# ducha-aiki/affnet

Hardware: NVIDIA H100
Metric: Mpix/s end-to-end HesAffNet(+OriNet)+HardNet (higher is better)
Workload: dtype fp16 operands (fp16 residual planes: AffNet/OriNet weights+activations, HardNet layer 2-3 weights), fp32 accumulate; stencils fp32

## Files before the change

affnet_b200/csrc/tcx_conv.cuh:

```cuda
#pragma once
#include <cuda_bf16.h>

#include "tc_conv.cuh"

#ifndef AG_CONV_PINGPONG
#define AG_CONV_PINGPONG 1
#endif

namespace ag {
namespace tcx {

using namespace ag::tc;

constexpr int XORDER = 5;

enum { CT_TOTAL, CT_WAIT_FULL, CT_TURN, CT_ISSUE, CT_MMA_WAIT, CT_EPILOGUE, CT_WG_BAR, CT_WAIT_EMPTY, CT_OTHER, CT_STATES };
#ifdef AG_CONV_TIMELINE
constexpr int CT_CTAS = 4, CT_LAUNCHES = 16, CT_EVENTS = 2048;
__device__ unsigned long long g_conv_tl[CT_LAUNCHES][CT_CTAS][9][CT_STATES];
__device__ unsigned long long g_conv_ev[CT_LAUNCHES][2][CT_EVENTS][3];
__device__ int g_conv_tl_launch[CT_CTAS];
struct ConvTimeline {
    unsigned long long t[CT_STATES];
    long long start, mark;
    int slot, warp, n_ev;
    __device__ static void claim(int* s_slot) {
        if (threadIdx.x == 0)
            *s_slot = (blockIdx.y == 0 && blockIdx.x < CT_CTAS) ? min(atomicAdd(&g_conv_tl_launch[blockIdx.x], 1), CT_LAUNCHES) : CT_LAUNCHES;
    }
    __device__ void init(const int* s_slot) {
        for (int i = 0; i < CT_STATES; i++) t[i] = 0;
        slot = *s_slot; warp = threadIdx.x >> 5; n_ev = 0;
        start = mark = clock64();
    }
    __device__ void lap(int state) { const long long now = clock64(); t[state] += (unsigned long long)(now - mark); mark = now; }
    __device__ void event(int k) {
        if (blockIdx.x == 0 && slot < CT_LAUNCHES && (threadIdx.x & 127) == 0 && n_ev < CT_EVENTS) g_conv_ev[slot][warp >> 2][n_ev][k] = (unsigned long long)mark;
        if (k == 2) n_ev++;
    }
    __device__ void finish() {
        t[CT_TOTAL] = (unsigned long long)(clock64() - start);
        if ((threadIdx.x & 31) == 0 && slot < CT_LAUNCHES)
            for (int i = 0; i < CT_STATES; i++) g_conv_tl[slot][blockIdx.x][warp][i] = t[i];
    }
};
#else
struct ConvTimeline {
    __device__ static void claim(int*) {}
    __device__ void init(const int*) {}
    __device__ void lap(int) {}
    __device__ void event(int) {}
    __device__ void finish() {}
};
#endif

enum XLayout { L_S2_16 = 0, L_S1_16 = 1, L_S2_8P = 2, L_S1_8P = 3, L_HEAD = 4 };

__device__ __forceinline__ void bulk_g2s_mc(void* dst, const void* src, uint32_t bytes, uint64_t* bar, uint16_t mask) {
    asm volatile("cp.async.bulk.shared::cluster.global.mbarrier::complete_tx::bytes.multicast::cluster [%0], [%1], %2, [%3], %4;" ::"r"(smem_u32(dst)),
                 "l"(src), "r"(bytes), "r"(smem_u32(bar)), "h"(mask)
                 : "memory");
}
__device__ __forceinline__ void mbar_arrive_cluster(uint64_t* bar, uint32_t cta) {
    asm volatile("{\n .reg .b32 ra;\n mapa.shared::cluster.u32 ra, %0, %1;\n mbarrier.arrive.release.cta.shared::cluster.b64 _, [ra];\n}\n" ::"r"(smem_u32(bar)), "r"(cta)
                 : "memory");
}
__device__ __forceinline__ void cluster_sync() {
    asm volatile("barrier.cluster.arrive.release.aligned;\n barrier.cluster.wait.acquire.aligned;" ::: "memory");
}

template <int BF>
__device__ __forceinline__ uint32_t pack2(float a, float b) {
    if (BF) { const __nv_bfloat162 h = __floats2bfloat162_rn(a, b); return *reinterpret_cast<const uint32_t*>(&h); }
    const __half2 h = __floats2half2_rn(a, b);
    return *reinterpret_cast<const uint32_t*>(&h);
}
template <int BF>
__device__ __forceinline__ float2 unpack2(uint32_t u) {
    if (BF) return make_float2(__uint_as_float(u << 16), __uint_as_float(u & 0xFFFF0000u));
    return __half22float2(*reinterpret_cast<const __half2*>(&u));
}
template <int LO, int BF = 0>
__device__ __forceinline__ void split_pack8(const float* v, uint4& hi, uint4& lo) {
    uint32_t h[4], l[4];
#pragma unroll
    for (int i = 0; i < 4; i++) {
        h[i] = pack2<BF>(v[2 * i], v[2 * i + 1]);
        if (LO) {
            const float2 f = unpack2<BF>(h[i]);
            l[i] = pack2<BF>(v[2 * i] - f.x, v[2 * i + 1] - f.y);
        } else l[i] = 0;
    }
    hi = make_uint4(h[0], h[1], h[2], h[3]);
    lo = make_uint4(l[0], l[1], l[2], l[3]);
}

template <int LO, int BF = 0>
__device__ __forceinline__ void split_pack2(float v0, float v1, uint32_t& hi, uint32_t& lo) {
    hi = pack2<BF>(v0, v1);
    if (LO) {
        const float2 f = unpack2<BF>(hi);
        lo = pack2<BF>(v0 - f.x, v1 - f.y);
    } else lo = 0;
}

__host__ __device__ constexpr int layout_slots(int lay) { return lay == L_S2_16 ? 1024 : lay == L_S1_16 ? 256 : lay == L_S2_8P ? 512 : 128; }
__host__ __device__ constexpr int layout_pair(int lay) { return (lay == L_S2_8P || lay == L_S1_8P) ? 1 : 0; }
__host__ __device__ constexpr int rpos(int x) { return (x & 1) * 8 + (x >> 1); }
__host__ __device__ constexpr int ppos(int x, int p) { return (x & 1) * 8 + p * 4 + (x >> 1); }
__host__ __device__ constexpr int layout_slot(int lay, int y, int x, int p) {
    return lay == L_S2_16 ? ((y & 1) * 2 + (x & 1)) * 256 + (y >> 1) * 16 + rpos(x >> 1)
         : lay == L_S1_16 ? y * 16 + rpos(x)
         : lay == L_S2_8P ? ((y & 1) * 2 + (x & 1)) * 128 + (y >> 1) * 16 + ppos(x >> 1, p)
                          : y * 16 + ppos(x, p);
}

template <int H, int STRIDE>
struct XIn {
    static constexpr int HOUT = H / STRIDE;
    static constexpr int PAIR = (HOUT == 8) ? 1 : 0;
    static constexpr int W = HOUT;
    static constexpr int RW = W * (1 + PAIR);
    static constexpr int TILES = HOUT * RW / 128;
    static constexpr int NPLANES = (STRIDE == 1) ? 1 : 4;
    static constexpr int DATA = HOUT * RW;
    static constexpr int PLANE = DATA + RW;
    static constexpr int SLOT_STAGE = NPLANES * PLANE;
    static constexpr int LAYOUT = (STRIDE == 2) ? (PAIR ? L_S2_8P : L_S2_16) : (PAIR ? L_S1_8P : L_S1_16);
    static_assert(HOUT == 8 || HOUT == 16 || HOUT == 32, "map sizes of the three nets");
    static_assert(!(STRIDE == 1 && H == 32), "the 32x32 stride-1 layer lives in tcx_first.cuh");
};

struct XArgs {
    const __half* in;
    void* out;
    const __half* wpk;
    const float* bias;
    float inv_scale;
    int n, group;
    const int* count;
};

template <int CIN, int COUT, int H, int STRIDE, int NSPLIT, int STAGES, int OUT, int SA, int SW, int OSA>
struct XCfg {
    using In = XIn<H, STRIDE>;
    static constexpr int CO = COUT, STRD = STRIDE, OUTL = OUT, SPLIT_A = SA, SPLIT_W = SW, SPLIT_O = OSA;
    static constexpr int KC = CIN / 8, NT = COUT / NSPLIT, HOUT = In::HOUT;
    static constexpr int G = KC * (1 + SA);
    static constexpr int GS = STAGES * In::SLOT_STAGE + (STRIDE == 1 ? In::RW : 0);
    static constexpr int ACCW = 3 * NT;
    static constexpr int BLOCKS = 2 * In::TILES;
    static constexpr uint32_t W_BYTES = 9u * CIN * NT * 2u * (1 + SW);
    static constexpr uint32_t IN_BYTES = (uint32_t)G * GS * 16u;
    static constexpr uint32_t HI_IN_BYTES = (uint32_t)KC * In::NPLANES * In::DATA * 16u;
    static constexpr uint32_t UNIT_IN_BYTES = HI_IN_BYTES * (1 + SA);
    static constexpr int THREADS = 288;
    static constexpr size_t SMEM = 1024 + (size_t)W_BYTES + IN_BYTES;
    static constexpr size_t HI_OUT_BYTES = (size_t)(COUT / 8) * layout_slots(OUT) * 16;
    static constexpr size_t UNIT_OUT_BYTES = (OUT == L_HEAD) ? 0 : HI_OUT_BYTES * (1 + OSA);
    static constexpr int NR1 = (1 + SW) * 3 * NT;
    static constexpr int NRO = (1 + SW) * 2 * NT, NRE = (1 + SW) * NT;
    static_assert(CIN % 16 == 0 && NT % 16 == 0 && ACCW <= 256, "wgmma shape");
    static_assert(In::W == 8 || In::W == 16, "a warp's 16 accumulator rows hold whole image rows");
    static_assert(SA <= 1 && SW <= 1 && OSA <= 1, "split-precision switches are 0 | 1");
    static_assert(2 * STAGES + 1 <= 60, "barrier area");
    static_assert(SMEM <= 232448, "shared memory budget");
    static_assert(GS < 16384, "leading-byte offset field");
    static_assert(OUT == L_HEAD || layout_pair(OUT) || !In::PAIR, "a pair layer writes pair layouts or the head operand");
};

__device__ __forceinline__ float frag_left_even(float v1, int lane) { return __shfl_sync(0xffffffffu, v1, (lane + 28) & 31); }
__device__ __forceinline__ float frag_right_odd(float v0, int lane) { return __shfl_sync(0xffffffffu, v0, (lane + 4) & 31); }

__device__ __forceinline__ bool xpatch_valid(const XArgs& a, int pi) { return pi < a.n && (a.count == nullptr || (pi % a.group) < a.count[pi / a.group]); }

template <class Cfg, int BF>
__device__ __forceinline__ void xconv_block_issue(float* d, uint32_t a_t, uint32_t w_base) {
    using In = typename Cfg::In;
    constexpr int KC = Cfg::KC, NT = Cfg::NT, GS = Cfg::GS, RW = In::RW, SA = Cfg::SPLIT_A, SW = Cfg::SPLIT_W;
    constexpr uint32_t LBO_A = ((uint32_t)GS) << 16;
    wgmma_fence();
    if (Cfg::STRD == 1) {
#pragma unroll
        for (int dy = 0; dy < 3; dy++) {
#pragma unroll
            for (int j = 0; j < KC / 2; j++) {
                const uint32_t ahi = ((a_t + (uint32_t)(dy * RW + 2 * j * GS)) & 0x3FFFu) | LBO_A;
                const uint32_t alo = ((a_t + (uint32_t)(dy * RW + (KC + 2 * j) * GS)) & 0x3FFFu) | LBO_A;
                const uint32_t blk = w_base + (uint32_t)((dy * (KC / 2) + j) * 2 * Cfg::NR1);
                const uint32_t bhi = (blk & 0x3FFFu) | ((uint32_t)Cfg::NR1 << 16), blo = ((blk + 3 * NT) & 0x3FFFu) | ((uint32_t)Cfg::NR1 << 16);
                Wgmma<3 * NT, BF>::mma(d, desc64(ahi), desc64(bhi), (dy | j) != 0);
                if (SW) Wgmma<3 * NT, BF>::mma(d, desc64(ahi), desc64(blo), 1);
                if (SA) Wgmma<3 * NT, BF>::mma(d, desc64(alo), desc64(bhi), 1);
            }
        }
    } else {
#pragma unroll
        for (int dy = 0; dy < 3; dy++) {
            constexpr int PL = In::PLANE;
            const int py = (dy == 1) ? 0 : 1, ro = (dy == 0) ? 0 : 1;
#pragma unroll
            for (int j = 0; j < KC / 2; j++) {
                const uint32_t blk = w_base + (uint32_t)((dy * (KC / 2) + j) * 2 * (Cfg::NRO + Cfg::NRE));
                const uint32_t bo_hi = (blk & 0x3FFFu) | ((uint32_t)Cfg::NRO << 16), bo_lo = ((blk + 2 * NT) & 0x3FFFu) | ((uint32_t)Cfg::NRO << 16);
                const uint32_t be = blk + 2 * Cfg::NRO;
                const uint32_t be_hi = (be & 0x3FFFu) | ((uint32_t)Cfg::NRE << 16), be_lo = ((be + NT) & 0x3FFFu) | ((uint32_t)Cfg::NRE << 16);
                const uint32_t ao = a_t + (uint32_t)((py * 2 + 1) * PL + ro * RW);
                const uint32_t ao_hi = ((ao + (uint32_t)(2 * j * GS)) & 0x3FFFu) | LBO_A, ao_lo = ((ao + (uint32_t)((KC + 2 * j) * GS)) & 0x3FFFu) | LBO_A;
                Wgmma<2 * NT, BF>::mma(d, desc64(ao_hi), desc64(bo_hi), (dy | j) != 0);
                if (SW) Wgmma<2 * NT, BF>::mma(d, desc64(ao_hi), desc64(bo_lo), 1);
                if (SA) Wgmma<2 * NT, BF>::mma(d, desc64(ao_lo), desc64(bo_hi), 1);
                const uint32_t ae = a_t + (uint32_t)((py * 2 + 0) * PL + ro * RW);
                const uint32_t ae_hi = ((ae + (uint32_t)(2 * j * GS)) & 0x3FFFu) | LBO_A, ae_lo = ((ae + (uint32_t)((KC + 2 * j) * GS)) & 0x3FFFu) | LBO_A;
                Wgmma<NT, BF>::mma(d + NT, desc64(ae_hi), desc64(be_hi), (dy | j) != 0);
                if (SW) Wgmma<NT, BF>::mma(d + NT, desc64(ae_hi), desc64(be_lo), 1);
                if (SA) Wgmma<NT, BF>::mma(d + NT, desc64(ae_lo), desc64(be_hi), 1);
            }
        }
    }
    wgmma_commit();
}
template <class Cfg, int BF>
__device__ __forceinline__ void xconv_block_epilogue(const float* d, const XArgs& a, const float* s_bias, int u, int b, int split, int wq, int lane) {
    using In = typename Cfg::In;
    constexpr int NT = Cfg::NT, HOUT = Cfg::HOUT, W = In::W, PAIR = In::PAIR, COUT = Cfg::CO, OUT = Cfg::OUTL, OSA = Cfg::SPLIT_O;
    unsigned char* obase[2];
    bool ok[2];
    size_t lo_off = 0;
    const int i = lane >> 2, xi = PAIR ? (i & 3) : i;
    const bool has_l0 = xi > 0, has_r1 = xi < W / 2 - 1;
    static_assert(W == 16 || PAIR, "neighbour-paired row groups: 16 pixels, or 8 of each patch of a pair");
#pragma unroll
    for (int h = 0; h < 2; h++) {
        const int y = b * 4 + wq, x = 2 * xi + h, pi = PAIR ? 2 * u + (i >> 2) : u;
        ok[h] = xpatch_valid(a, pi);
        if (OUT == L_HEAD) {
            obase[h] = reinterpret_cast<unsigned char*>(a.out) + (((size_t)(pi >> 7) * (HOUT * HOUT * COUT / 8) + (size_t)(y * HOUT + x) * (COUT / 8)) * 128 + (pi & 127)) * 16;
            lo_off = (size_t)((a.n + 127) >> 7) * (HOUT * HOUT * COUT / 8) * 128 * 16;
        } else {
            const int ou = layout_pair(OUT) ? (pi >> 1) : pi;
            obase[h] = reinterpret_cast<unsigned char*>(a.out) + (size_t)ou * Cfg::UNIT_OUT_BYTES + (size_t)layout_slot(OUT, y, x, pi & 1) * 16;
            lo_off = (size_t)(COUT / 8) * layout_slots(OUT) * 16;
        }
    }
#pragma unroll
    for (int j = 0; j < NT / 8; j++) {
        const int c = j * 8 + 2 * (lane & 3);
        float v[2][2];
#pragma unroll
        for (int e = 0; e < 2; e++) {
            const float c00 = d[4 * j + e], c01 = d[4 * j + 2 + e];
            const float c10 = d[4 * (j + NT / 8) + e], c11 = d[4 * (j + NT / 8) + 2 + e];
            const float c20 = d[4 * (j + 2 * NT / 8) + e], c21 = d[4 * (j + 2 * NT / 8) + 2 + e];
            const float l0 = frag_left_even(c01, lane);
            float acc0, acc1;
            if (Cfg::STRD == 1) {
                const float r1 = frag_right_odd(c20, lane);
                const float t0 = c21 + c10, t1 = has_r1 ? r1 + c11 : c11;
                acc0 = has_l0 ? l0 + t0 : t0;
                acc1 = c00 + t1;
            } else {
                const float t0 = c10 + c20, t1 = c11 + c21;
                acc0 = has_l0 ? l0 + t0 : t0;
                acc1 = c00 + t1;
            }
            v[0][e] = fmaxf(fmaf(acc0, a.inv_scale, s_bias[c + e]), 0.f);
            v[1][e] = fmaxf(fmaf(acc1, a.inv_scale, s_bias[c + e]), 0.f);
        }
        const int ch = split * NT + c;
        const size_t goff = ((OUT == L_HEAD) ? (size_t)(ch / 8) * 128 * 16 : (size_t)(ch / 8) * layout_slots(OUT) * 16) + (ch & 7) * 2;
#pragma unroll
        for (int h = 0; h < 2; h++) {
            if (!ok[h]) continue;
            uint32_t hi, lo;
            split_pack2<OSA, BF>(v[h][0], v[h][1], hi, lo);
            *reinterpret_cast<uint32_t*>(obase[h] + goff) = hi;
            if (OSA) *reinterpret_cast<uint32_t*>(obase[h] + lo_off + goff) = lo;
        }
    }
}

template <int CIN, int COUT, int H, int STRIDE, int NSPLIT, int STAGES, int OUT, int SA, int SW, int OSA, int BF = 0, int MC = 0, int PPS = 0>
__global__ void __launch_bounds__(288, 1) tcx_conv_kernel(const XArgs a) {
    static_assert(MC == 0 || NSPLIT == 2, "multicast pairs the two channel-split CTAs");
    using Cfg = XCfg<CIN, COUT, H, STRIDE, NSPLIT, STAGES, OUT, SA, SW, OSA>;
    using In = typename Cfg::In;
    constexpr int ACCW = Cfg::ACCW, BLOCKS = Cfg::BLOCKS, GS = Cfg::GS, RW = In::RW;
    constexpr int PAIR = In::PAIR;
    constexpr bool PP = AG_CONV_PINGPONG && PPS;
    extern __shared__ __align__(1024) unsigned char smem[];
    uint64_t* full = reinterpret_cast<uint64_t*>(smem);
    uint64_t* empty = full + STAGES;
    uint64_t* wbar = empty + STAGES;
    float* s_bias = reinterpret_cast<float*>(smem + 512);
    unsigned char* sW = smem + 1024;
    unsigned char* sIn = sW + Cfg::W_BYTES;

    const int warp = threadIdx.x >> 5, lane = threadIdx.x & 31;
    const int split = blockIdx.y;
    const int n_units = PAIR ? (a.n + 1) >> 1 : a.n;

    int* s_tl_slot = reinterpret_cast<int*>(smem + 496);

    if (threadIdx.x < Cfg::NT) s_bias[threadIdx.x] = a.bias[split * Cfg::NT + threadIdx.x];
    if (threadIdx.x == 0) {
        for (int s = 0; s < STAGES; s++) { mbar_init(&full[s], 1); mbar_init(&empty[s], (PP ? 8 : 2) * (1 + MC)); }
        mbar_init(wbar, 1);
        asm volatile("fence.mbarrier_init.release.cluster;" ::: "memory");
    }
    ConvTimeline::claim(s_tl_slot);
    for (int i = threadIdx.x; i < (int)(Cfg::IN_BYTES / 16); i += blockDim.x) reinterpret_cast<uint4*>(sIn)[i] = make_uint4(0, 0, 0, 0);
    asm volatile("fence.proxy.async.shared::cta;" ::: "memory");
    __syncthreads();
    if (MC) cluster_sync();
    ConvTimeline tl;
    tl.init(s_tl_slot);
    auto release = [&](uint64_t* e) {
        if (MC) { mbar_arrive_cluster(e, 0); mbar_arrive_cluster(e, 1); }
        else mbar_arrive(e);
    };

    auto uvalid = [&](int u) -> bool { return PAIR ? (xpatch_valid(a, 2 * u) || xpatch_valid(a, 2 * u + 1)) : xpatch_valid(a, u); };

    if (warp == 8) {
        if (lane == 0) {
            mbar_expect_tx(wbar, Cfg::W_BYTES);
            bulk_g2s(sW, reinterpret_cast<const unsigned char*>(a.wpk) + (size_t)split * Cfg::W_BYTES, Cfg::W_BYTES, wbar);
            int it = 0;
            for (int u = blockIdx.x; u < n_units; u += gridDim.x) {
                if (!uvalid(u)) continue;
                const int s = it % STAGES;
                tl.lap(CT_OTHER);
                mbar_wait(&empty[s], ((it / STAGES) & 1) ^ 1);
                tl.lap(CT_WAIT_EMPTY);
                mbar_expect_tx(&full[s], Cfg::UNIT_IN_BYTES);
                const unsigned char* gsrc = reinterpret_cast<const unsigned char*>(a.in) + (size_t)u * Cfg::UNIT_IN_BYTES;
#pragma unroll 1
                for (int g = 0; g < Cfg::G; g++)
#pragma unroll
                    for (int pl = 0; pl < In::NPLANES; pl++) {
                        unsigned char* dst = sIn + ((size_t)g * GS + (size_t)s * In::SLOT_STAGE + (size_t)pl * In::PLANE + RW) * 16;
                        const unsigned char* srcp = gsrc + ((size_t)g * In::NPLANES + pl) * In::DATA * 16;
                        if (MC) { if (((g * In::NPLANES + pl) & 1) == split) bulk_g2s_mc(dst, srcp, In::DATA * 16u, &full[s], (uint16_t)3); }
                        else bulk_g2s(dst, srcp, In::DATA * 16u, &full[s]);
                    }
                it++;
            }
            tl.lap(CT_OTHER);
            if (MC) {
                for (int k = 0; k < STAGES && k < it; k++) { const int j = it - 1 - k; mbar_wait(&empty[j % STAGES], (j / STAGES) & 1); }
            }
            tl.lap(CT_WAIT_EMPTY);
        }
    } else if (warp < 8) {
        const int wg = warp >> 2, wq = warp & 3;
        mbar_wait(wbar, 0);
        const uint32_t w_base = smem_u32(sW) >> 4;
        const uint32_t in_base = smem_u32(sIn) >> 4;
        int it = 0;
        for (int u = blockIdx.x; u < n_units; u += gridDim.x) {
            if (!uvalid(u)) continue;
            const int s = it % STAGES;
            tl.lap(CT_OTHER);
            mbar_wait(&full[s], (it / STAGES) & 1);
            tl.lap(CT_WAIT_FULL);
            const uint32_t st_base = in_base + (uint32_t)(s * In::SLOT_STAGE);
#pragma unroll 1
            for (int b = wg; b < BLOCKS; b += 2) {
                float d[ACCW / 2];
                if (PP && (wg == 1 || it > 0 || b > 0)) bar_sync(XORDER + wg, 256);
                tl.lap(CT_TURN);
                tl.event(0);
                xconv_block_issue<Cfg, BF>(d, st_base + (uint32_t)(b * 64), w_base);
                if (PP) asm volatile("bar.arrive %0, 256;" ::"r"(XORDER + (wg ^ 1)) : "memory");
                tl.lap(CT_ISSUE);
                wgmma_wait<0>();
                wgmma_reg_fence<ACCW / 2>(d);
                tl.lap(CT_MMA_WAIT);
                tl.event(1);
                if (PP && b + 2 >= BLOCKS && lane == 0) release(&empty[s]);
                xconv_block_epilogue<Cfg, BF>(d, a, s_bias, u, b, split, wq, lane);
                tl.lap(CT_EPILOGUE);
                tl.event(2);
            }
            if (!PP) {
                bar_sync(3 + wg, 128);
                tl.lap(CT_WG_BAR);
                if ((threadIdx.x & 127) == 0) release(&empty[s]);
            }
            it++;
        }
        if (PP && wg == 0 && it > 0) bar_sync(XORDER, 256);
        tl.lap(CT_OTHER);
    }
    tl.finish();
    __syncthreads();
    if (MC) cluster_sync();
}

}
}
```

affnet_b200/csrc/tcx_first.cuh:

```cuda
#pragma once
#include "tcx_conv.cuh"

#ifdef AG_FIRST_TIMELINE
#define AG_TL(state, ...) do { const long long t_ = clock64(); __VA_ARGS__; tl[state] += (unsigned long long)(clock64() - t_); } while (0)
#else
#define AG_TL(state, ...) do { __VA_ARGS__; } while (0)
#endif

namespace ag {
namespace tcx {

enum { TL_TOTAL, TL_WAIT_P, TL_ISSUE, TL_MMA_WAIT, TL_WG_BAR, TL_STAGE_BAR, TL_PBUILD, TL_STATES };
#ifdef AG_FIRST_TIMELINE
constexpr int TL_CTAS = 4, TL_LAUNCHES = 8;
__device__ unsigned long long g_first_tl[TL_LAUNCHES][TL_CTAS][16][TL_STATES];
__device__ int g_first_tl_launch[TL_CTAS];
#endif

__device__ __forceinline__ void stmatrix_x4(const void* row, uint32_t r0, uint32_t r1, uint32_t r2, uint32_t r3) {
    asm volatile("stmatrix.sync.aligned.m8n8.x4.shared.b16 [%0], {%1, %2, %3, %4};" ::"r"(smem_u32(row)), "r"(r0), "r"(r1), "r"(r2), "r"(r3)
                 : "memory");
}

template <int C1, int COUT, int SA, int SW, int OSA, int L3 = 0>
struct XFirstCfg {
    using X3 = XCfg<COUT, 2 * COUT, 32, 2, 1, 1, L_S1_16, 1, 1, 1>;
    static constexpr int KC = C1 / 8, NT = COUT;
    static constexpr int BLOCKS = 16;
    static constexpr int NPIXP = 18 * 32;
    static constexpr int SX = 1200;
    static constexpr int S1 = (C1 == 16) ? 1 : 0;
    static constexpr int ACC1 = 32;
    static constexpr int ACCW = 3 * NT;
    static constexpr int G = KC * (1 + SA);
    static constexpr int SLOT_STAGE = 1024 + 32;
    static constexpr int NSTAGE = L3 ? 1 : 2;
    static constexpr int GS = NSTAGE * SLOT_STAGE + 32;
    static constexpr int NR = (1 + SW) * 3 * NT;
    static constexpr uint32_t W_BYTES = 9u * C1 * NT * 2u * (1 + SW);
    static constexpr uint32_t IN_BYTES = (uint32_t)G * GS * 16u;
    static constexpr uint32_t W1_BYTES = 2u * 2u * C1 * 16;
    static constexpr uint32_t P_BYTES = 2u * 2u * NPIXP * 16;
    static constexpr uint32_t XCH_BYTES = 2u * 2u * 4u * 2u * NT * 4u;
    static constexpr uint32_t W3_BYTES = L3 ? X3::W_BYTES : 0u;
    static constexpr uint32_t IN3_BYTES = L3 ? X3::IN_BYTES : 0u;
    static constexpr size_t SMEM = 1024 + (size_t)W_BYTES + W3_BYTES + IN_BYTES + IN3_BYTES + P_BYTES + W1_BYTES + 2 * SX * 4 + 256 + XCH_BYTES;
    static constexpr size_t HI_OUT_BYTES = (size_t)(COUT / 8) * 1024 * 16;
    static constexpr size_t UNIT_OUT_BYTES = HI_OUT_BYTES * (1 + OSA);
    static constexpr int THREADS = 512;
    static constexpr int REG_PRODUCER = 96, REG_CONSUMER = 160;
    static_assert(256 * (REG_PRODUCER + REG_CONSUMER) <= 65536 && REG_PRODUCER % 8 == 0 && REG_CONSUMER % 8 == 0, "register split");
    static_assert(BLOCKS % 4 == 0 && (!L3 || X3::BLOCKS == 4), "two blocks in flight per warpgroup: an even count of blocks each");
    static_assert(C1 % 16 == 0 && NT % 16 == 0 && ACCW <= 256, "shape");
    static_assert(SA <= 1 && SW <= 1 && OSA <= 1, "split-precision switches are 0 | 1");
    static_assert(!L3 || (OSA == 1 && X3::NT <= 32), "layer 3 reads hi + lo planes; its bias fits smem[640, 768)");
    static_assert(C1 == 16 || C1 == 32, "layer-1 accumulator width");
    static_assert(SA || KC % 2 == 0, "layer-1 epilogue: one stmatrix.x4 per channel group (hi + lo) or per two (hi only)");
    static_assert(SMEM <= 232448, "shared memory budget");
};

template <int C1, int COUT, int SA, int SW, int OSA, int BF = 0, int L3 = 0>
__global__ void __launch_bounds__(512, 1) tcx_first_kernel(const XArgs a, const FirstSrc src, const XArgs a3) {
    using Cfg = XFirstCfg<C1, COUT, SA, SW, OSA, L3>;
    using X3 = typename Cfg::X3;
    constexpr int KC = Cfg::KC, NT = Cfg::NT, ACCW = Cfg::ACCW, NPIXP = Cfg::NPIXP, SX = Cfg::SX, GS = Cfg::GS;
    extern __shared__ __align__(1024) unsigned char smem[];
    uint64_t* wbar = reinterpret_cast<uint64_t*>(smem);
    uint64_t* p_full = wbar + 1;
    uint64_t* p_empty = p_full + 2;
    float* s_bias1 = reinterpret_cast<float*>(smem + 384);
    float* s_bias = reinterpret_cast<float*>(smem + 512);
    float* s_bias3 = reinterpret_cast<float*>(smem + 640);
    unsigned char* sW = smem + 1024;
    unsigned char* sW3 = sW + Cfg::W_BYTES;
    unsigned char* sIn = sW3 + Cfg::W3_BYTES;
    unsigned char* sIn3 = sIn + Cfg::IN_BYTES;
    unsigned char* sP = sIn3 + Cfg::IN3_BYTES;
    unsigned char* sW1 = sP + Cfg::P_BYTES;
    float* s_x = reinterpret_cast<float*>(sW1 + Cfg::W1_BYTES);
    float* s_red = s_x + 2 * SX;
    float* s_xch = s_red + 64;

    const int warp = threadIdx.x >> 5, lane = threadIdx.x & 31;
    auto valid = [&](int pi) -> bool { return a.count == nullptr || (pi % a.group) < a.count[pi / a.group]; };
    auto next_valid = [&](int pi) -> int {
        while (pi < a.n && !valid(pi)) pi += gridDim.x;
        return pi;
    };

    if (threadIdx.x < NT) s_bias[threadIdx.x] = a.bias[threadIdx.x];
    if (threadIdx.x < C1) s_bias1[threadIdx.x] = src.b1[threadIdx.x];
    if (L3 && threadIdx.x < X3::NT) s_bias3[threadIdx.x] = a3.bias[threadIdx.x];
    if (threadIdx.x == 0) {
        mbar_init(wbar, 1);
        for (int hh = 0; hh < 2; hh++) { mbar_init(&p_full[hh], 256); mbar_init(&p_empty[hh], 2); }
        asm volatile("fence.mbarrier_init.release.cluster;" ::: "memory");
    }
#ifdef AG_FIRST_TIMELINE
    int* s_tl_slot = reinterpret_cast<int*>(smem + 128);
    if (threadIdx.x == 0) *s_tl_slot = blockIdx.x < TL_CTAS ? min(atomicAdd(&g_first_tl_launch[blockIdx.x], 1), TL_LAUNCHES) : TL_LAUNCHES;
    unsigned long long tl[TL_STATES] = {};
#endif
    for (int i = threadIdx.x; i < 2 * 2 * C1 * 8; i += blockDim.x) {
        const int e = i & 7, co = (i >> 3) % C1, part = (i / (8 * C1)) & 1, ch = i / (8 * C1 * 2);
        const int dy = ch == 0 ? (e >> 2) : 2, dx = e & 3;
        float v = 0.f;
        if (dx < 3 && (ch == 0 || e < 4)) {
            const float wv = src.w1[(dy * 3 + dx) * C1 + co] * src.w1_scale;
            const float hi = unpack2<BF>(pack2<BF>(wv, 0.f)).x;
            v = part == 0 ? hi : wv - hi;
        }
        reinterpret_cast<unsigned short*>(sW1)[i] = (unsigned short)(pack2<BF>(v, 0.f) & 0xFFFFu);
    }
    for (int i = threadIdx.x; i < (int)((Cfg::IN_BYTES + Cfg::IN3_BYTES + Cfg::P_BYTES) / 16); i += blockDim.x) reinterpret_cast<uint4*>(sIn)[i] = make_uint4(0, 0, 0, 0);
    for (int i = threadIdx.x; i < 2 * SX; i += blockDim.x) s_x[i] = 0.f;
    asm volatile("fence.proxy.async.shared::cta;" ::: "memory");
    __syncthreads();
#ifdef AG_FIRST_TIMELINE
    const long long tl_start = clock64();
#endif

    if (warp >= 8) {
        asm volatile("setmaxnreg.inc.sync.aligned.u32 %0;" ::"n"(Cfg::REG_CONSUMER));
        const int wg = (warp - 8) >> 2, wq = warp & 3;
        if (threadIdx.x == 256) {
            mbar_expect_tx(wbar, Cfg::W_BYTES + Cfg::W3_BYTES);
            bulk_g2s(sW, a.wpk, Cfg::W_BYTES, wbar);
            if (L3) bulk_g2s(sW3, a3.wpk, Cfg::W3_BYTES, wbar);
        }
        mbar_wait(wbar, 0);
        const uint32_t w_base = smem_u32(sW) >> 4, in_base = smem_u32(sIn) >> 4;
        const uint32_t w3_base = smem_u32(sW3) >> 4, in3_base = smem_u32(sIn3) >> 4;
        const uint32_t w1_lo = desc_lo(smem_u32(sW1), 2 * C1 * 16u);
        const uint32_t p_lo = desc_lo(smem_u32(sP), 2 * 32 * 16u);
        constexpr uint32_t LBO_A = ((uint32_t)GS) << 16;
        auto l1_issue = [&](float* d1, int hh, int b) {
            const uint32_t alo = p_lo + (uint32_t)(hh * 2 * NPIXP + (b & 7) * 64);
            wgmma_fence();
            if (Cfg::S1) {
                Wgmma<2 * C1, BF>::mma(d1, desc64(alo), desc64(w1_lo), 0);
                Wgmma<C1, BF>::mma(d1, desc64(alo + (uint32_t)NPIXP), desc64(w1_lo), 1);
            } else {
                Wgmma<C1, BF>::mma(d1, desc64(alo), desc64(w1_lo), 0);
                Wgmma<C1, BF>::mma(d1, desc64(alo + (uint32_t)NPIXP), desc64(w1_lo), 1);
                Wgmma<C1, BF>::mma(d1, desc64(alo), desc64(w1_lo + (uint32_t)C1), 1);
            }
            wgmma_commit();
        };
        auto l1_epilogue = [&](float* d1, unsigned char* st, int b) {
            wgmma_reg_fence<Cfg::ACC1 / 2>(d1);
            uint32_t hi[KC][2], lo[KC][2];
#pragma unroll
            for (int h = 0; h < 2; h++) {
#pragma unroll
                for (int j = 0; j < KC; j++) {
                    const int c = j * 8 + 2 * (lane & 3);
                    float v0 = d1[4 * j + 2 * h], v1 = d1[4 * j + 2 * h + 1];
                    if (Cfg::S1) { v0 += d1[4 * (j + 2) + 2 * h]; v1 += d1[4 * (j + 2) + 2 * h + 1]; }
                    v0 = fmaxf(fmaf(v0, src.w1_inv, s_bias1[c]), 0.f);
                    v1 = fmaxf(fmaf(v1, src.w1_inv, s_bias1[c + 1]), 0.f);
                    split_pack2<SA, BF>(v0, v1, hi[j][h], lo[j][h]);
                }
            }
            const int mx = lane >> 3;
            const int slot = b * 64 + wq * 16 + (lane & 7) + 8 * (mx & 1) + 32;
#pragma unroll
            for (int j = 0; j < KC; j += SA ? 1 : 2) {
                if constexpr (SA) stmatrix_x4(st + ((size_t)((mx >> 1) * KC + j) * GS + slot) * 16, hi[j][0], hi[j][1], lo[j][0], lo[j][1]);
                else stmatrix_x4(st + ((size_t)(j + (mx >> 1)) * GS + slot) * 16, hi[j][0], hi[j][1], hi[j + 1][0], hi[j + 1][1]);
            }
        };
        auto l1_block = [&](int k) -> int { return (k >> 2) * 8 + wg + 2 * (k & 3); };
        int it = 0, nblk = 0;
        for (int pi = next_valid(blockIdx.x); pi < a.n; pi = next_valid(pi + gridDim.x), it++) {
            const int s = L3 ? 0 : (it & 1);
            unsigned char* st = sIn + (size_t)s * Cfg::SLOT_STAGE * 16;
            float d1[2][Cfg::ACC1 / 2];
            AG_TL(TL_WAIT_P, mbar_wait(&p_full[0], it & 1));
            AG_TL(TL_ISSUE, l1_issue(d1[0], 0, l1_block(0)));
#pragma unroll
            for (int k = 0; k < 8; k++) {
                if (k < 7) {
                    if (k == 3) AG_TL(TL_WAIT_P, mbar_wait(&p_full[1], it & 1));
                    AG_TL(TL_ISSUE, l1_issue(d1[(k + 1) & 1], (k + 1) >> 2, l1_block(k + 1)));
                    AG_TL(TL_MMA_WAIT, wgmma_wait<1>());
                } else {
                    AG_TL(TL_MMA_WAIT, wgmma_wait<0>());
                }
                l1_epilogue(d1[k & 1], st, l1_block(k));
            }
            asm volatile("fence.proxy.async.shared::cta;" ::: "memory");
            AG_TL(TL_STAGE_BAR, bar_sync(2, 256));
            if ((threadIdx.x & 127) == 0) { mbar_arrive(&p_empty[0]); mbar_arrive(&p_empty[1]); }
            unsigned char* outp = L3 ? nullptr : reinterpret_cast<unsigned char*>(a.out) + (size_t)pi * Cfg::UNIT_OUT_BYTES;
            const uint32_t st_base = in_base + (uint32_t)(s * Cfg::SLOT_STAGE);
            auto l2_issue = [&](float* d, int b) {
                const uint32_t a_t = st_base + (uint32_t)(b * 64);
                wgmma_fence();
#pragma unroll
                for (int dy = 0; dy < 3; dy++) {
#pragma unroll
                    for (int j = 0; j < KC / 2; j++) {
                        const uint32_t ahi = ((a_t + (uint32_t)(dy * 32 + 2 * j * GS)) & 0x3FFFu) | LBO_A;
                        const uint32_t alo = ((a_t + (uint32_t)(dy * 32 + (KC + 2 * j) * GS)) & 0x3FFFu) | LBO_A;
                        const uint32_t blk = w_base + (uint32_t)((dy * (KC / 2) + j) * 2 * Cfg::NR);
                        const uint32_t bhi = (blk & 0x3FFFu) | ((uint32_t)Cfg::NR << 16), blo = ((blk + 3 * NT) & 0x3FFFu) | ((uint32_t)Cfg::NR << 16);
                        Wgmma<3 * NT, BF>::mma(d, desc64(ahi), desc64(bhi), (dy | j) != 0);
                        if (SW) Wgmma<3 * NT, BF>::mma(d, desc64(ahi), desc64(blo), 1);
                        if (SA) Wgmma<3 * NT, BF>::mma(d, desc64(alo), desc64(bhi), 1);
                    }
                }
                wgmma_commit();
            };
            auto l2_epilogue = [&](float* d, int b, int nb) {
                wgmma_reg_fence<ACCW / 2>(d);
                float* xw = s_xch + (size_t)((wg * 2 + (nb & 1)) * 4) * 2 * NT;
                if (lane >= 28) {
#pragma unroll
                    for (int j = 0; j < NT / 8; j++) {
                        const int c = j * 8 + 2 * (lane & 3);
                        xw[(wq * 2 + 0) * NT + c] = d[4 * j + 2]; xw[(wq * 2 + 0) * NT + c + 1] = d[4 * j + 3];
                    }
                }
                if (lane < 4) {
#pragma unroll
                    for (int j = 0; j < NT / 8; j++) {
                        const int c = j * 8 + 2 * (lane & 3);
                        xw[(wq * 2 + 1) * NT + c] = d[4 * (j + 2 * NT / 8)]; xw[(wq * 2 + 1) * NT + c + 1] = d[4 * (j + 2 * NT / 8) + 1];
                    }
                }
                AG_TL(TL_WG_BAR, bar_sync(3 + wg, 128));
                const int y0 = (b * 64 + wq * 16) >> 5;
                const int x0 = (wq & 1) * 16 + 2 * (lane >> 2);
                const bool first8 = lane < 16;
                const float m0 = (first8 && x0 == 0) ? 0.f : 1.f, m1 = (!first8 && x0 + 1 == 31) ? 0.f : 1.f;
                const bool from_prev = (wq & 1) && lane < 4, from_next = !(wq & 1) && lane >= 28;
                size_t s3 = 0;
                if (L3) {
                    using In3 = typename X3::In;
                    const int mx = lane >> 3;
                    const int slot = layout_slot(L_S2_16, y0, (wq & 1) * 16 + 2 * (lane & 7) + (mx & 1), 0);
                    s3 = (size_t)(mx >> 1) * X3::KC * X3::GS + (size_t)(slot / In3::DATA) * In3::PLANE + In3::RW + slot % In3::DATA;
                }
#pragma unroll
                for (int j = 0; j < NT / 8; j++) {
                    const int c = j * 8 + 2 * (lane & 3);
                    float v[2][2];
#pragma unroll
                    for (int e = 0; e < 2; e++) {
                        const float c00 = d[4 * j + e], c01 = d[4 * j + 2 + e];
                        const float c10 = d[4 * (j + NT / 8) + e], c11 = d[4 * (j + NT / 8) + 2 + e];
                        const float c20 = d[4 * (j + 2 * NT / 8) + e], c21 = d[4 * (j + 2 * NT / 8) + 2 + e];
                        float l0 = frag_left_even(c01, lane), r1 = frag_right_odd(c20, lane);
                        const float l1 = c00, r0 = c21;
                        if (from_prev) l0 = xw[((wq - 1) * 2 + 0) * NT + c + e];
                        if (from_next) r1 = xw[((wq + 1) * 2 + 1) * NT + c + e];
                        const float acc0 = fmaf(first8 ? l0 : r0, m0, (first8 ? r0 : l0) + c10);
                        const float acc1 = fmaf(first8 ? l1 : r1, m1, (first8 ? r1 : l1) + c11);
                        v[0][e] = fmaxf(fmaf(acc0, a.inv_scale, s_bias[c + e]), 0.f);
                        v[1][e] = fmaxf(fmaf(acc1, a.inv_scale, s_bias[c + e]), 0.f);
                    }
                    uint32_t hi[2], lo[2];
#pragma unroll
                    for (int h = 0; h < 2; h++) split_pack2<OSA, BF>(v[h][0], v[h][1], hi[h], lo[h]);
                    if (L3) {
                        stmatrix_x4(sIn3 + ((size_t)j * X3::GS + s3) * 16, hi[0], hi[1], lo[0], lo[1]);
                    } else {
#pragma unroll
                        for (int h = 0; h < 2; h++) {
                            const int slot = layout_slot(L_S2_16, y0, x0 + h, 0);
                            const size_t goff = (size_t)(c / 8) * 1024 * 16;
                            *reinterpret_cast<uint32_t*>(outp + goff + (size_t)slot * 16 + (c & 7) * 2) = hi[h];
                            if (OSA) *reinterpret_cast<uint32_t*>(outp + (size_t)(COUT / 8) * 1024 * 16 + goff + (size_t)slot * 16 + (c & 7) * 2) = lo[h];
                        }
                    }
                }
            };
            float d[2][ACCW / 2];
            AG_TL(TL_ISSUE, l2_issue(d[0], wg));
#pragma unroll
            for (int k = 0; k < Cfg::BLOCKS / 2; k++) {
                if (k + 1 < Cfg::BLOCKS / 2) {
                    AG_TL(TL_ISSUE, l2_issue(d[(k + 1) & 1], wg + 2 * (k + 1)));
                    AG_TL(TL_MMA_WAIT, wgmma_wait<1>());
                } else {
                    AG_TL(TL_MMA_WAIT, wgmma_wait<0>());
                }
                l2_epilogue(d[k & 1], wg + 2 * k, nblk + k);
            }
            nblk += Cfg::BLOCKS / 2;
            if (L3) {
                asm volatile("fence.proxy.async.shared::cta;" ::: "memory");
                AG_TL(TL_STAGE_BAR, bar_sync(2, 256));
                float d3[2][X3::ACCW / 2];
                AG_TL(TL_ISSUE, xconv_block_issue<X3, BF>(d3[0], in3_base + (uint32_t)(wg * 64), w3_base));
                AG_TL(TL_ISSUE, xconv_block_issue<X3, BF>(d3[1], in3_base + (uint32_t)((wg + 2) * 64), w3_base));
                AG_TL(TL_MMA_WAIT, wgmma_wait<1>());
                wgmma_reg_fence<X3::ACCW / 2>(d3[0]);
                xconv_block_epilogue<X3, BF>(d3[0], a3, s_bias3, pi, wg, 0, wq, lane);
                AG_TL(TL_MMA_WAIT, wgmma_wait<0>());
                wgmma_reg_fence<X3::ACCW / 2>(d3[1]);
                xconv_block_epilogue<X3, BF>(d3[1], a3, s_bias3, pi, wg + 2, 0, wq, lane);
            }
        }
    } else {
        asm volatile("setmaxnreg.dec.sync.aligned.u32 %0;" ::"n"(Cfg::REG_PRODUCER));
        const int pw = warp;
        const int pt = pw * 32 + lane;
        float tp[4][4], fx[4], fy[4];
        auto pix_of = [&](int k) -> int { return (pw * 4 + (lane >> 3)) * 32 + k * 8 + (lane & 7); };
        auto issue_fetch = [&](int pi) {
            if (src.patches != nullptr) {
                const float* pp = src.patches + (size_t)pi * 1024;
#pragma unroll
                for (int k = 0; k < 4; k++) { tp[k][0] = pp[pix_of(k)]; tp[k][1] = tp[k][2] = tp[k][3] = 0.f; fx[k] = 0.f; fy[k] = 0.f; }
            } else {
                const int b = pi / src.cap;
                const int o = min(max(src.oct[pi], 0), src.geom.n_octaves - 1), l = min(max(src.lvl[pi], 0), src.geom.n_levels - 1);
                const int h = src.geom.h[o], w = src.geom.w[o];
                const float* img = src.pyr + src.geom.off[o][l] + (size_t)b * h * w;
                const float* Lf = src.lafs + (size_t)pi * 6;
#pragma unroll
                for (int k = 0; k < 4; k++) {
                    const int p = pix_of(k);
                    float px, py;
                    laf_sample_xy(Lf, h, w, p >> 5, p & 31, 1.0f / 32.0f, px, py);
                    bilinear_taps(img, h, w, px, py, tp[k], fx[k], fy[k]);
                }
            }
        };
        int pi = next_valid(blockIdx.x);
        if (pi < a.n) issue_fetch(pi);
        int it = 0;
        while (pi < a.n) {
            float* sx = s_x + (it & 1) * SX;
            float* red = s_red + (it & 1) * 16;
            float v[4];
#pragma unroll
            for (int k = 0; k < 4; k++) v[k] = bilinear_combine(tp[k], fx[k], fy[k]);
            const int pn = next_valid(pi + gridDim.x);
            if (pn < a.n) issue_fetch(pn);
            float sm = (v[0] + v[1]) + (v[2] + v[3]);
            for (int o = 16; o > 0; o >>= 1) sm += __shfl_xor_sync(0xffffffffu, sm, o);
            if (lane == 0) red[pw * 2] = sm;
            AG_TL(TL_WG_BAR, asm volatile("bar.sync 1, 256;" ::: "memory"));
            const float mean = (((red[0] + red[2]) + (red[4] + red[6])) + ((red[8] + red[10]) + (red[12] + red[14]))) / 1024.f;
            float qs = 0.f;
#pragma unroll
            for (int k = 0; k < 4; k++) { const float d = v[k] - mean; qs = fmaf(d, d, qs); }
            for (int o = 16; o > 0; o >>= 1) qs += __shfl_xor_sync(0xffffffffu, qs, o);
            if (lane == 0) red[pw * 2 + 1] = qs;
            AG_TL(TL_WG_BAR, asm volatile("bar.sync 1, 256;" ::: "memory"));
            const float inv = 1.f / (sqrtf((((red[1] + red[3]) + (red[5] + red[7])) + ((red[9] + red[11]) + (red[13] + red[15]))) / 1023.f) + 1e-7f);
#pragma unroll
            for (int k = 0; k < 4; k++) { const int p = pix_of(k); sx[((p >> 5) + 1) * 34 + (p & 31) + 1] = (v[k] - mean) * inv; }
            AG_TL(TL_WG_BAR, asm volatile("bar.sync 1, 256;" ::: "memory"));
#pragma unroll 1
            for (int hh = 0; hh < 2; hh++) {
                AG_TL(TL_WAIT_P, mbar_wait(&p_empty[hh], (it & 1) ^ 1));
#ifdef AG_FIRST_TIMELINE
                const long long tb = clock64();
#endif
                unsigned char* ph = sP + (size_t)hh * 2 * NPIXP * 16;
#pragma unroll 1
                for (int s0 = pt; s0 < NPIXP; s0 += 256) {
                    const float* rowp = sx + (hh * 16 + (s0 >> 5)) * 34 + (s0 & 16) + 2 * (s0 & 7) + ((s0 >> 3) & 1);
                    float xv[8];
#pragma unroll
                    for (int e = 0; e < 4; e++) { xv[e] = rowp[e]; xv[4 + e] = rowp[34 + e]; }
                    uint4 hi, lo;
                    split_pack8<1, BF>(xv, hi, lo);
                    *reinterpret_cast<uint4*>(ph + (size_t)s0 * 16) = hi;
                    *reinterpret_cast<uint4*>(ph + (size_t)(NPIXP + s0) * 16) = lo;
                }
                asm volatile("fence.proxy.async.shared::cta;" ::: "memory");
                mbar_arrive(&p_full[hh]);
#ifdef AG_FIRST_TIMELINE
                tl[TL_PBUILD] += (unsigned long long)(clock64() - tb);
#endif
            }
            it++;
            pi = pn;
        }
    }
#ifdef AG_FIRST_TIMELINE
    tl[TL_TOTAL] = (unsigned long long)(clock64() - tl_start);
    if (lane == 0 && *s_tl_slot < TL_LAUNCHES)
        for (int i = 0; i < TL_STATES; i++) g_first_tl[*s_tl_slot][blockIdx.x][warp][i] = tl[i];
#endif
}

}
}
```

Measured before the change: 669.6.

## Stage fused layer-3 epilogue through shared memory and bulk-copy to global

The fused layer-3 epilogue now writes its results with stmatrix into free layer-1 input slots in shared memory, then issues cp.async.bulk shared-to-global copies of 1 KiB chunks instead of scattered 4-byte global stores. This is meant to cut the cost of uncoalesced global stores and to let the output writes run asynchronously alongside the next patch's work. Reusing the staging buffer requires waiting on the bulk reads plus a warpgroup barrier before the next patch's layer-1 epilogue overwrites it, which adds synchronisation.

```diff
diff --git a/affnet_b200/csrc/tcx_conv.cuh b/affnet_b200/csrc/tcx_conv.cuh
--- a/affnet_b200/csrc/tcx_conv.cuh
+++ b/affnet_b200/csrc/tcx_conv.cuh
@@ -172,6 +172,17 @@
 __device__ __forceinline__ float frag_left_even(float v1, int lane) { return __shfl_sync(0xffffffffu, v1, (lane + 28) & 31); }
 __device__ __forceinline__ float frag_right_odd(float v0, int lane) { return __shfl_sync(0xffffffffu, v0, (lane + 4) & 31); }
 
+__device__ __forceinline__ void stmatrix_x4(const void* row, uint32_t r0, uint32_t r1, uint32_t r2, uint32_t r3) {
+    asm volatile("stmatrix.sync.aligned.m8n8.x4.shared.b16 [%0], {%1, %2, %3, %4};" ::"r"(smem_u32(row)), "r"(r0), "r"(r1), "r"(r2), "r"(r3)
+                 : "memory");
+}
+__device__ __forceinline__ void bulk_s2g(void* dst, const void* src, uint32_t bytes) {
+    asm volatile("cp.async.bulk.global.shared::cta.bulk_group [%0], [%1], %2;" ::"l"(dst), "r"(smem_u32(src)), "r"(bytes) : "memory");
+}
+__device__ __forceinline__ void bulk_commit() { asm volatile("cp.async.bulk.commit_group;" ::: "memory"); }
+__device__ __forceinline__ void bulk_wait_read_all() { asm volatile("cp.async.bulk.wait_group.read 0;" ::: "memory"); }
+__device__ __forceinline__ void bulk_wait_all() { asm volatile("cp.async.bulk.wait_group 0;" ::: "memory"); }
+
 __device__ __forceinline__ bool xpatch_valid(const XArgs& a, int pi) { return pi < a.n && (a.count == nullptr || (pi % a.group) < a.count[pi / a.group]); }
 
 template <class Cfg, int BF>
@@ -277,6 +288,47 @@
             *reinterpret_cast<uint32_t*>(obase[h] + goff) = hi;
             if (OSA) *reinterpret_cast<uint32_t*>(obase[h] + lo_off + goff) = lo;
         }
+    }
+}
+
+template <class Cfg, int BF, class Stg>
+__device__ __forceinline__ void xconv_block_epilogue_staged(const float* d, const XArgs& a, const float* s_bias, Stg stg, int wq, int lane) {
+    using In = typename Cfg::In;
+    constexpr int NT = Cfg::NT;
+    static_assert(Cfg::OUTL == L_S1_16 && NT == Cfg::CO && In::W == 16 && !In::PAIR, "whole unit, rows of 16 pixels, 64 contiguous slots per block");
+    static_assert(Cfg::SPLIT_O == 1, "hi + lo planes: one stmatrix.x4 per channel group");
+    const int i = lane >> 2;
+    const bool has_l0 = i > 0, has_r1 = i < In::W / 2 - 1;
+    const int mx = lane >> 3;
+    const int row = wq * 16 + (mx & 1) * 8 + (lane & 7);
+#pragma unroll
+    for (int j = 0; j < NT / 8; j++) {
+        const int c = j * 8 + 2 * (lane & 3);
+        float v[2][2];
+#pragma unroll
+        for (int e = 0; e < 2; e++) {
+            const float c00 = d[4 * j + e], c01 = d[4 * j + 2 + e];
+            const float c10 = d[4 * (j + NT / 8) + e], c11 = d[4 * (j + NT / 8) + 2 + e];
+            const float c20 = d[4 * (j + 2 * NT / 8) + e], c21 = d[4 * (j + 2 * NT / 8) + 2 + e];
+            const float l0 = frag_left_even(c01, lane);
+            float acc0, acc1;
+            if (Cfg::STRD == 1) {
+                const float r1 = frag_right_odd(c20, lane);
+                const float t0 = c21 + c10, t1 = has_r1 ? r1 + c11 : c11;
+                acc0 = has_l0 ? l0 + t0 : t0;
+                acc1 = c00 + t1;
+            } else {
+                const float t0 = c10 + c20, t1 = c11 + c21;
+                acc0 = has_l0 ? l0 + t0 : t0;
+                acc1 = c00 + t1;
+            }
+            v[0][e] = fmaxf(fmaf(acc0, a.inv_scale, s_bias[c + e]), 0.f);
+            v[1][e] = fmaxf(fmaf(acc1, a.inv_scale, s_bias[c + e]), 0.f);
+        }
+        uint32_t hi[2], lo[2];
+#pragma unroll
+        for (int h = 0; h < 2; h++) split_pack2<1, BF>(v[h][0], v[h][1], hi[h], lo[h]);
+        stmatrix_x4(stg(j + (mx >> 1) * (NT / 8)) + row * 16, hi[0], hi[1], lo[0], lo[1]);
     }
 }
 
diff --git a/affnet_b200/csrc/tcx_first.cuh b/affnet_b200/csrc/tcx_first.cuh
--- a/affnet_b200/csrc/tcx_first.cuh
+++ b/affnet_b200/csrc/tcx_first.cuh
@@ -16,11 +16,6 @@
 __device__ unsigned long long g_first_tl[TL_LAUNCHES][TL_CTAS][16][TL_STATES];
 __device__ int g_first_tl_launch[TL_CTAS];
 #endif
-
-__device__ __forceinline__ void stmatrix_x4(const void* row, uint32_t r0, uint32_t r1, uint32_t r2, uint32_t r3) {
-    asm volatile("stmatrix.sync.aligned.m8n8.x4.shared.b16 [%0], {%1, %2, %3, %4};" ::"r"(smem_u32(row)), "r"(r0), "r"(r1), "r"(r2), "r"(r3)
-                 : "memory");
-}
 
 template <int C1, int COUT, int SA, int SW, int OSA, int L3 = 0>
 struct XFirstCfg {
@@ -56,6 +51,7 @@
     static_assert(!L3 || (OSA == 1 && X3::NT <= 32), "layer 3 reads hi + lo planes; its bias fits smem[640, 768)");
     static_assert(C1 == 16 || C1 == 32, "layer-1 accumulator width");
     static_assert(SA || KC % 2 == 0, "layer-1 epilogue: one stmatrix.x4 per channel group (hi + lo) or per two (hi only)");
+    static_assert(!L3 || 2 * X3::CO / 8 * 2 <= KC * (1 + SA) * 8, "layer-3 staging: two blocks' 1 KiB chunks per warpgroup fit in its layer-1 blocks");
     static_assert(SMEM <= 232448, "shared memory budget");
 };
 
@@ -171,6 +167,10 @@
             }
         };
         auto l1_block = [&](int k) -> int { return (k >> 2) * 8 + wg + 2 * (k & 3); };
+        constexpr int OG3 = L3 ? 2 * X3::CO / 8 : 1;
+        auto stg3 = [&](int n) -> unsigned char* {
+            return sIn + ((size_t)(n % Cfg::G) * GS + 32 + (size_t)(wg + 2 * (n / Cfg::G)) * 64) * 16;
+        };
         int it = 0, nblk = 0;
         for (int pi = next_valid(blockIdx.x); pi < a.n; pi = next_valid(pi + gridDim.x), it++) {
             const int s = L3 ? 0 : (it & 1);
@@ -186,6 +186,10 @@
                     AG_TL(TL_MMA_WAIT, wgmma_wait<1>());
                 } else {
                     AG_TL(TL_MMA_WAIT, wgmma_wait<0>());
+                }
+                if (L3 && k == 0 && it > 0) {
+                    if (lane == 0) bulk_wait_read_all();
+                    AG_TL(TL_WG_BAR, bar_sync(3 + wg, 128));
                 }
                 l1_epilogue(d1[k & 1], st, l1_block(k));
             }
@@ -295,14 +299,24 @@
                 float d3[2][X3::ACCW / 2];
                 AG_TL(TL_ISSUE, xconv_block_issue<X3, BF>(d3[0], in3_base + (uint32_t)(wg * 64), w3_base));
                 AG_TL(TL_ISSUE, xconv_block_issue<X3, BF>(d3[1], in3_base + (uint32_t)((wg + 2) * 64), w3_base));
+                auto l3_block = [&](float* d3b, int b, int q) {
+                    wgmma_reg_fence<X3::ACCW / 2>(d3b);
+                    xconv_block_epilogue_staged<X3, BF>(d3b, a3, s_bias3, [&](int g) { return stg3(q * OG3 + g); }, wq, lane);
+                    asm volatile("fence.proxy.async.shared::cta;" ::: "memory");
+                    AG_TL(TL_WG_BAR, bar_sync(3 + wg, 128));
+                    if (lane == 0 && wq < OG3) {
+                        unsigned char* o3 = reinterpret_cast<unsigned char*>(a3.out) + (size_t)pi * X3::UNIT_OUT_BYTES + (size_t)b * 64 * 16;
+                        for (int g = wq; g < OG3; g += 4) bulk_s2g(o3 + (size_t)g * 256 * 16, stg3(q * OG3 + g), 1024u);
+                        bulk_commit();
+                    }
+                };
                 AG_TL(TL_MMA_WAIT, wgmma_wait<1>());
-                wgmma_reg_fence<X3::ACCW / 2>(d3[0]);
-                xconv_block_epilogue<X3, BF>(d3[0], a3, s_bias3, pi, wg, 0, wq, lane);
+                l3_block(d3[0], wg, 0);
                 AG_TL(TL_MMA_WAIT, wgmma_wait<0>());
-                wgmma_reg_fence<X3::ACCW / 2>(d3[1]);
-                xconv_block_epilogue<X3, BF>(d3[1], a3, s_bias3, pi, wg + 2, 0, wq, lane);
+                l3_block(d3[1], wg + 2, 1);
             }
         }
+        if (L3 && lane == 0) bulk_wait_all();
     } else {
         asm volatile("setmaxnreg.dec.sync.aligned.u32 %0;" ::"n"(Cfg::REG_PRODUCER));
         const int pw = warp;
```

After: 682.0 (median of 6 runs). 1.8% higher.
